# TorchIO-project/torchio

Measured on NVIDIA H100. Metric: augmented voxels/sec on 256^3 fp32 Compose pipeline, higher is better.
Workload: dtype f32

## Files before the change

### torchio_b200/csrc/fused_intensity.cu

```cuda
#include "common.cuh"
#include "tma.cuh"

namespace tio {

__device__ __forceinline__ float rician(float x, float n1, float n2) {
  float s = __fadd_rn(x, n1);
  return sqrtf(__fadd_rn(__fmul_rn(s, s), __fmul_rn(n2, n2)));
}


__device__ __forceinline__ uint4 philox4x32_10(uint4 ctr, uint2 key) {
  const uint32_t M0 = 0xD2511F53u, M1 = 0xCD9E8D57u, W0 = 0x9E3779B9u, W1 = 0xBB67AE85u;
#pragma unroll
  for (int r = 0; r < 7; ++r) {
    uint32_t hi0 = __umulhi(M0, ctr.x), lo0 = M0 * ctr.x;
    uint32_t hi1 = __umulhi(M1, ctr.z), lo1 = M1 * ctr.z;
    ctr = make_uint4(hi1 ^ ctr.y ^ key.x, lo1, hi0 ^ ctr.w ^ key.y, lo0);
    key.x += W0;
    key.y += W1;
  }
  return ctr;
}

__device__ __forceinline__ void box_muller(uint32_t a, uint32_t b, float& n0, float& n1) {
// ... 532 lines not shown
        } else {
          z1[0] = nz.z[flat];
          if (nz.rician) z2[0] = nz.z2[flat];
        }
      } else {
        const uint2 key = make_uint2((uint32_t)nz.philox_seed, (uint32_t)(nz.philox_seed >> 32));
        const uint64_t gidx = (uint64_t)(flat / V);
        uint4 rr = philox4x32_10(make_uint4((uint32_t)gidx, (uint32_t)(gidx >> 32), 0u, 0x5eedu), key);
        float nn[4];
        box_muller(rr.x, rr.y, nn[0], nn[1]);
        box_muller(rr.z, rr.w, nn[2], nn[3]);
#pragma unroll
        for (int q = 0; q < V; ++q) z1[q] = nn[q];
        if (nz.rician) {
          uint4 r2 = philox4x32_10(make_uint4((uint32_t)gidx, (uint32_t)(gidx >> 32), 1u, 0x5eedu), key);
          box_muller(r2.x, r2.y, nn[0], nn[1]);
          box_muller(r2.z, r2.w, nn[2], nn[3]);
#pragma unroll
          for (int q = 0; q < V; ++q) z2[q] = nn[q];
        }
      }
#pragma unroll
      for (int q = 0; q < V; ++q) {
        float n1 = __fadd_rn(mu, __fmul_rn(sd, z1[q]));
        if (nz.rician) v[q] = rician(v[q], n1, __fadd_rn(mu, __fmul_rn(sd, z2[q])));
        else v[q] = __fadd_rn(v[q], n1);
      }
    }
    if (gamma) {
#pragma unroll
      for (int q = 0; q < V; ++q) v[q] = signed_pow(v[q], gam);
    }
    if (V == 4) *(float4*)(y + o) = make_float4(v[0], v[1], v[2], v[3]);
    else y[o] = v[0];
  };

  if (r == 0) {
    for (int i = 0; i < I; ++i) {
      float v[V];
      load_plane(i, v);
      finish(i, v);
    }
    return;
  }

  float* mine = ring + tid * V;
  const int slot_stride = 256 * V;
  auto put = [&](int pos, const float* v) {
    int s = pos % W; if (s < 0) s += W;
    if (V == 4) *(float4*)(mine + s * slot_stride) = make_float4(v[0], v[1], v[2], v[3]);
    else mine[s * slot_stride] = v[0];
  };
  float first[V];
  load_plane(0, first);
  for (int p = -r; p <= 0; ++p) put(p, first);
  float last[V];
#pragma unroll
  for (int q = 0; q < V; ++q) last[q] = first[q];
  for (int p = 1; p < I + r; ++p) {
    if (p < I) load_plane(p, last);
    put(p, last);
    const int o = p - r;
    if (o < 0) continue;
    float acc[V];
#pragma unroll
    for (int q = 0; q < V; ++q) acc[q] = 0.0f;
    int s = (o - r) % W; if (s < 0) s += W;
    for (int t = 0; t < W; ++t) {
      const float tp = tapi[R - r + t];
      if (V == 4) {
        float4 w4 = *(const float4*)(mine + s * slot_stride);
        acc[0] = __fmaf_rn(tp, w4.x, acc[0]); acc[1] = __fmaf_rn(tp, w4.y, acc[1]);
        acc[2] = __fmaf_rn(tp, w4.z, acc[2]); acc[3] = __fmaf_rn(tp, w4.w, acc[3]);
      } else {
        acc[0] = __fmaf_rn(tp, mine[s * slot_stride], acc[0]);
      }
      if (++s == W) s = 0;
    }
    finish(o, acc);
  }
}

constexpr int M6_PF = 8;

template <bool HAS_BIAS, bool EPI>
__global__ void __launch_bounds__(256, EPI ? 1 : 2)
march6_kernel(const float* __restrict__ src, float* __restrict__ dst, int B, int C, int I, int J,
              int K, BlurArgs bl, BiasArgs bi, NoiseArgs nz, const float* __restrict__ gamma) {
  extern __shared__ __align__(16) float smem[];
  constexpr int W = 2 * F_R + 1;
  const int bc = blockIdx.z;
  const int b = bc / C;
  const int tid = threadIdx.y * blockDim.x + threadIdx.x;
  const int k = (blockIdx.x * blockDim.x + threadIdx.x) * 4;
  const int j = blockIdx.y * blockDim.y + threadIdx.y;
  const int64_t n = (int64_t)I * J * K;
  const float* x = src + (int64_t)bc * n;
  float* y = dst + (int64_t)bc * n;

  const int r = bl.taps ? bl.radius[0 * B + b] : 0;
  float* tapi = smem;
  float* g = smem + 16;
  const int ns = HAS_BIAS ? bi.si * bi.sj * bi.sk : 0;
  const bool bias_on = HAS_BIAS && !(bi.identity && bi.identity[b]);
  if (tid < W) {
    const int off = tid - F_R;
    tapi[tid] = (r > 0 && off >= -r && off <= r) ? bl.taps[((int64_t)0 * B + b) * (2 * bl.R + 1) + bl.R + off] : 0.0f;
  }
  if (bias_on) {
    const float* gs = bi.coarse + (int64_t)bc * ns;
    for (int t = tid; t < ns; t += 256) g[t] = gs[t];
  }
  __syncthreads();
  if (k >= K || j >= J) return;

  const bool noise_on = EPI && nz.mode != 0 && (!nz.keep || nz.keep[b]);
  const float mu = (EPI && nz.mode) ? nz.mean[b] : 0.0f, sd = (EPI && nz.mode) ? nz.std[b] : 0.0f;
  const float gam = (EPI && gamma) ? gamma[b] : 1.0f;
  const int gamma_mode = !(EPI && gamma) || gam == 1.0f ? 0 : (gam > 0.0f ? 1 : 2);

  LerpAxis lj, lk[4];
  int o00[4], o01[4], o10[4], o11[4];
  int cur0 = -1, cur1 = -1;
  float r_lo[4], r_hi[4];
  if (bias_on) {
    lj = lerp_axis(bi.sc_j, bi.sj, j);
#pragma unroll
    for (int v = 0; v < 4; ++v) {
      lk[v] = lerp_axis(bi.sc_k, bi.sk, k + v);
      o00[v] = lj.i0 * bi.sk + lk[v].i0; o01[v] = lj.i0 * bi.sk + lk[v].i1;
      o10[v] = lj.i1 * bi.sk + lk[v].i0; o11[v] = lj.i1 * bi.sk + lk[v].i1;
    }
  }
  const int col = j * K + k;
  const int plane = J * K;

  float4* fifo = reinterpret_cast<float4*>(g + ((ns + 3) / 4) * 4) + tid;
  auto fifo_issue = [&](int pl) {
    if (pl < I) {
      const uint32_t sa = (uint32_t)__cvta_generic_to_shared(fifo + (pl & (M6_PF - 1)) * 256);
      asm volatile("cp.async.cg.shared.global [%0], [%1], 16;" ::"r"(sa), "l"(x + (int64_t)pl * plane + col) : "memory");
    }
    asm volatile("cp.async.commit_group;" ::: "memory");
  };
#pragma unroll
  for (int pl = 0; pl < M6_PF - 1; ++pl) fifo_issue(pl);

  auto load_plane = [&](int i, float* out) {
    fifo_issue(i + M6_PF - 1);
    asm volatile("cp.async.wait_group %0;" ::"n"(M6_PF - 1) : "memory");
    const float4 t = fifo[(i & (M6_PF - 1)) * 256];
    out[0] = t.x; out[1] = t.y; out[2] = t.z; out[3] = t.w;
    if (bias_on) {
      const LerpAxis li = lerp_axis(bi.sc_i, bi.si, i);
      if (li.i0 != cur0 || li.i1 != cur1) {
        const float* p0 = g + (li.i0 * bi.sj) * bi.sk;
        const float* p1 = g + (li.i1 * bi.sj) * bi.sk;
#pragma unroll
        for (int v = 0; v < 4; ++v) {
          const float a0 = lerp2(lk[v].l0, p0[o00[v]], lk[v].l1, p0[o01[v]]);
          const float a1 = lerp2(lk[v].l0, p0[o10[v]], lk[v].l1, p0[o11[v]]);
          r_lo[v] = lerp2(lj.l0, a0, lj.l1, a1);
          const float b0 = lerp2(lk[v].l0, p1[o00[v]], lk[v].l1, p1[o01[v]]);
          const float b1 = lerp2(lk[v].l0, p1[o10[v]], lk[v].l1, p1[o11[v]]);
          r_hi[v] = lerp2(lj.l0, b0, lj.l1, b1);
        }
        cur0 = li.i0; cur1 = li.i1;
      }
#pragma unroll
      for (int v = 0; v < 4; ++v) {
        const float f = expf(lerp2(li.l0, r_lo[v], li.l1, r_hi[v]));
        out[v] = bi.divide ? __fdiv_rn(out[v], f) : __fmul_rn(out[v], f);
      }
    }
  };

  auto finish = [&](int i, float* v) {
    const int64_t o = (int64_t)i * plane + col;
    if (EPI) {
      if (noise_on) {
        const int64_t flat = (int64_t)bc * n + o;
        float z1[4], z2[4];
        if (nz.mode == 1) {
          const float4 t = __ldcs((const float4*)(nz.z + flat));
          z1[0] = t.x; z1[1] = t.y; z1[2] = t.z; z1[3] = t.w;
          if (nz.rician) {
            const float4 u = __ldcs((const float4*)(nz.z2 + flat));
            z2[0] = u.x; z2[1] = u.y; z2[2] = u.z; z2[3] = u.w;
          }
        } else {
          const uint2 key = make_uint2((uint32_t)nz.philox_seed, (uint32_t)(nz.philox_seed >> 32));
          const uint64_t gidx = (uint64_t)(flat / 4);
          uint4 rr = philox4x32_10(make_uint4((uint32_t)gidx, (uint32_t)(gidx >> 32), 0u, 0x5eedu), key);
          box_muller(rr.x, rr.y, z1[0], z1[1]);
          box_muller(rr.z, rr.w, z1[2], z1[3]);
          if (nz.rician) {
            uint4 r2 = philox4x32_10(make_uint4((uint32_t)gidx, (uint32_t)(gidx >> 32), 1u, 0x5eedu), key);
            box_muller(r2.x, r2.y, z2[0], z2[1]);
            box_muller(r2.z, r2.w, z2[2], z2[3]);
          }
        }
#pragma unroll
        for (int q = 0; q < 4; ++q) {
          const float n1 = __fadd_rn(mu, __fmul_rn(sd, z1[q]));
          if (nz.rician) v[q] = rician(v[q], n1, __fadd_rn(mu, __fmul_rn(sd, z2[q])));
          else v[q] = __fadd_rn(v[q], n1);
        }
      }
      if (gamma_mode == 1) {
#pragma unroll
        for (int q = 0; q < 4; ++q) v[q] = signed_pow_pos(v[q], gam);
      } else if (gamma_mode == 2) {
#pragma unroll
        for (int q = 0; q < 4; ++q) v[q] = signed_pow(v[q], gam);
      }
    }
    *(float4*)(y + o) = make_float4(v[0], v[1], v[2], v[3]);
  };

  if (r == 0) {
    for (int i = 0; i < I; ++i) {
      float v[4];
      load_plane(i, v);
      finish(i, v);
    }
    return;
  }

  float tp[W];
#pragma unroll
  for (int t = 0; t < W; ++t) tp[t] = tapi[t];
  float ring[W][4];
  {
    float first[4];
// ... 51 lines not shown
  const int pos = (int)((e / s) % L);
  const float* x = src + (int64_t)bc * n + (e - pos * s);
  float acc;
  if (r == 0) {
    acc = x[pos * s];
  } else {
    acc = 0.0f;
    for (int t = 0; t <= 2 * r; ++t) {
      const int q = min(max(pos - r + t, 0), L - 1);
      acc = __fmaf_rn(taps_s[t], __ldg(x + q * s), acc);
    }
  }
  const int64_t flat = (int64_t)bc * n + e;
  if (HAS_EPI) {
    if (nz.mode != 0 && (!nz.keep || nz.keep[b])) {
      const float mu = nz.mean[b], sd = nz.std[b];
      float z1, z2 = 0.0f;
      if (nz.mode == 1) {
        z1 = nz.z[flat];
        if (nz.rician) z2 = nz.z2[flat];
      } else {
        const uint2 key = make_uint2((uint32_t)nz.philox_seed, (uint32_t)(nz.philox_seed >> 32));
        float unused;
        uint4 rr = philox4x32_10(make_uint4((uint32_t)flat, (uint32_t)((uint64_t)flat >> 32), 0u, 0x77ffu), key);
        box_muller(rr.x, rr.y, z1, unused);
        if (nz.rician) box_muller(rr.z, rr.w, z2, unused);
      }
      const float n1 = __fadd_rn(mu, __fmul_rn(sd, z1));
      acc = nz.rician ? rician(acc, n1, __fadd_rn(mu, __fmul_rn(sd, z2))) : __fadd_rn(acc, n1);
    }
    if (gamma) acc = signed_pow(acc, gamma[b]);
  }
  dst[flat] = acc;
}

static inline bool aligned16f(const void* p) { return ((uintptr_t)p & 15) == 0; }

static float up_scale(int n_in, int n_out) {
  if (n_in == n_out) return 1.0f;
  return n_out > 1 ? (float)(n_in - 1) / (float)(n_out - 1) : 0.0f;
}

template <int RMAX>
static int launch_jk(const float* src, float* dst, int B, int C, int I, int J, int K,
                     const BlurArgs& bl, const NoiseArgs& nz, const float* gamma, cudaStream_t st) {
  constexpr int ROWS = A_TJ + 2 * RMAX, COLS = A_TK + 2 * RMAX, PITCH = (COLS + 3) / 4 * 4 + 4;
  const size_t smem = (size_t)(ROWS * PITCH + ROWS * A_TK + 2 * (2 * RMAX + 1)) * sizeof(float);
  const int tiles_i = (I + A_PLANES - 1) / A_PLANES;
  dim3 grid((K + A_TK - 1) / A_TK, (J + A_TJ - 1) / A_TJ, B * C * tiles_i);
  if (nz.mode != 0 || gamma) {
    if (smem > 48 * 1024)
      cudaFuncSetAttribute(jk_kernel<RMAX, true>, cudaFuncAttributeMaxDynamicSharedMemorySize, (int)smem);
    jk_kernel<RMAX, true><<<grid, 256, smem, st>>>(src, dst, B, C, I, J, K, bl, nz, gamma);
  } else {
    if (smem > 48 * 1024)
      cudaFuncSetAttribute(jk_kernel<RMAX, false>, cudaFuncAttributeMaxDynamicSharedMemorySize, (int)smem);
    jk_kernel<RMAX, false><<<grid, 256, smem, st>>>(src, dst, B, C, I, J, K, bl, nz, gamma);
  }
  return 0;
}

static int launch_march(const float* cur, float* out, int B, int C, int I, int J, int K,
                        const BiasArgs& bi, const BlurArgs& ib, const NoiseArgs& nz1,
                        const float* gamma1, cudaStream_t st, const char* who) {
  {
    const bool vec = (K % 4 == 0) && aligned16f(cur) && aligned16f(out) &&
                     (nz1.mode != 1 || (aligned16f(nz1.z) && (!nz1.z2 || aligned16f(nz1.z2))));
    const int V = vec ? 4 : 1;
    dim3 block(64, 4);
    dim3 grid((K + 64 * V - 1) / (64 * V), (J + 3) / 4, B * C);
    TIO_CHECK_ARG(grid.y <= 65535, "%s: J too large", who);
    const int R = ib.taps ? ib.R : 0;
    const int ns = bi.coarse ? bi.si * bi.sj * bi.sk : 0;
    const size_t smem = ((size_t)((2 * R + 1 + 3) / 4 * 4) + (size_t)((ns + 3) / 4 * 4) +
                         (ib.taps ? (size_t)(2 * R + 1) * 256 * V : 0)) * sizeof(float);
#define TIO_LAUNCH_MARCH(VV, BB)                                                              \
  do {                                                                                        \
    if (smem > 48 * 1024)                                                                     \
      cudaFuncSetAttribute(march_kernel<VV, BB>, cudaFuncAttributeMaxDynamicSharedMemorySize, \
                           (int)smem);                                                        \
    march_kernel<VV, BB><<<grid, block, smem, st>>>(cur, out, B, C, I, J, K, ib, bi, nz1, gamma1); \
  } while (0)
    if (vec && R <= F_R) {
      const size_t smem6 = (size_t)(16 + (ns + 3) / 4 * 4) * sizeof(float) + (size_t)M6_PF * 256 * 16;
#define TIO_LAUNCH_MARCH6(BB, EE)                                                              \
  do {                                                                                         \
    if (smem6 > 48 * 1024)                                                                     \
      cudaFuncSetAttribute(march6_kernel<BB, EE>, cudaFuncAttributeMaxDynamicSharedMemorySize, \
                           (int)smem6);                                                        \
    march6_kernel<BB, EE><<<grid, block, smem6, st>>>(cur, out, B, C, I, J, K, ib, bi, nz1, gamma1); \
  } while (0)
      const bool epi = nz1.mode != 0 || gamma1 != nullptr;
      if (bi.coarse) { if (epi) TIO_LAUNCH_MARCH6(true, true); else TIO_LAUNCH_MARCH6(true, false); }
      else { if (epi) TIO_LAUNCH_MARCH6(false, true); else TIO_LAUNCH_MARCH6(false, false); }
#undef TIO_LAUNCH_MARCH6
    } else if (vec) { if (bi.coarse) TIO_LAUNCH_MARCH(4, true); else TIO_LAUNCH_MARCH(4, false); }
    else { if (bi.coarse) TIO_LAUNCH_MARCH(1, true); else TIO_LAUNCH_MARCH(1, false); }
#undef TIO_LAUNCH_MARCH
  }
  return 0;
}

static int wide_impl(const float* src, float* dst, float* scratch, int B, int C, int I, int J,
                     int K, const BiasArgs& bi, const BlurArgs& bl, int axes_mask,
                     const NoiseArgs& nz, const float* gamma, cudaStream_t st, const char* who) {
  TIO_CHECK_ARG(bl.R <= WIDE_RMAX, "%s: blur radius R=%d > %d unsupported", who, bl.R, WIDE_RMAX);
  int axes[3], na = 0;
  for (int a : {0, 2, 1})
    if (axes_mask & (1 << a)) axes[na++] = a;
  const int steps = na + (bi.coarse ? 1 : 0);
  TIO_CHECK_ARG(src != dst && (steps < 2 || (scratch && scratch != src && scratch != dst)),
                "%s: blur radius R=%d > 16 needs src != dst and a scratch buffer", who, bl.R);
  const int64_t n = (int64_t)I * J * K;
  TIO_CHECK_ARG((n + 255) / 256 <= 0x7fffffff, "%s: volume too large", who);
  const float* cur = src;
  int left = steps;
  auto next_out = [&]() { return (--left % 2 == 0) ? dst : scratch; };
  if (bi.coarse) {
    BlurArgs none = bl;
    none.taps = nullptr;
    float* out = next_out();
    if (launch_march(cur, out, B, C, I, J, K, bi, none, NoiseArgs{}, nullptr, st, who)) return 1;
    cur = out;
  }
  const size_t smem = (size_t)(2 * bl.R + 1) * sizeof(float);
  dim3 grid((unsigned)((n + 255) / 256), B * C);
  for (int s = 0; s < na; ++s) {
    float* out = next_out();
    if (s == na - 1 && (nz.mode != 0 || gamma))
      axis_kernel<true><<<grid, 256, smem, st>>>(cur, out, B, C, I, J, K, axes[s], bl, nz, gamma);
    else
      axis_kernel<false><<<grid, 256, smem, st>>>(cur, out, B, C, I, J, K, axes[s], bl, nz, gamma);
    cur = out;
  }
  TIO_CHECK_LAUNCH();
  return 0;
}

static int fused_impl(const float* src, float* dst, float* scratch, int B, int C, int I, int J,
                      int K, BiasArgs bi, BlurArgs bl, int axes_mask, NoiseArgs nz,
                      const float* gamma, cudaStream_t st, const char* who) {
  TIO_CHECK_ARG(src && dst, "%s: null src/dst", who);
  TIO_CHECK_ARG(B > 0 && C > 0 && I > 0 && J > 0 && K > 0, "%s: bad shape", who);
  TIO_CHECK_ARG((int64_t)B * C <= 65535, "%s: B*C must be <= 65535", who);
  if (!bl.taps) axes_mask = 0;
  TIO_CHECK_ARG(!bl.taps || (bl.radius && bl.R >= 0), "%s: blur radius table missing or R=%d < 0", who, bl.R);
  if (bi.coarse) {
    bi.sc_i = up_scale(bi.si, I); bi.sc_j = up_scale(bi.sj, J); bi.sc_k = up_scale(bi.sk, K);
    TIO_CHECK_ARG((size_t)bi.si * bi.sj * bi.sk * 4 <= 64 * 1024, "%s: coarse bias grid too large", who);
  }
  if (axes_mask != 0 && bl.R > 16)
    return wide_impl(src, dst, scratch, B, C, I, J, K, bi, bl, axes_mask, nz, gamma, st, who);
  const bool need_jk = (axes_mask & 6) != 0;
  TIO_CHECK_ARG(!need_jk || (scratch && src != dst && scratch != src && scratch != dst),
                "%s: blur along J/K needs a scratch buffer and src != dst", who);
  TIO_CHECK_ARG(!((axes_mask & 1) && src == dst && !need_jk), "%s: blur along I needs src != dst", who);
  const bool need_i = (axes_mask & 1) != 0;
  const bool need_march = !need_jk || need_i || bi.coarse != nullptr;
  const float* cur = src;
  if (need_jk) {
    const int64_t tiles = (int64_t)B * C * ((I + A_PLANES - 1) / A_PLANES);
    TIO_CHECK_ARG(tiles <= 65535, "%s: batch too large for the blur grid", who);
  }
  if (need_march) {
    BlurArgs ib = bl;
    if (!need_i) ib.taps = nullptr;
    float* out = need_jk ? scratch : dst;
    if (launch_march(cur, out, B, C, I, J, K, bi, ib, need_jk ? NoiseArgs{} : nz,
                     need_jk ? nullptr : gamma, st, who))
      return 1;
    cur = out;
  }
  if (need_jk) {
    const bool tma_ok = bl.R <= F_R && (K % 4 == 0) && aligned16f(cur) && (int64_t)B * C * I < (1ll << 31);
    EncodeTiledFn encode = tma_ok ? encode_tiled_fn() : nullptr;
    CUtensorMap tm;
    bool have_map = false;
    if (encode) {
      const cuuint64_t gdim[3] = {(cuuint64_t)K, (cuuint64_t)J, (cuuint64_t)B * C * I};
      const cuuint64_t gstride[2] = {(cuuint64_t)K * 4, (cuuint64_t)J * K * 4};
      const cuuint32_t bdim[3] = {(cuuint32_t)F_COLS, (cuuint32_t)F_ROWS, 1};
      const cuuint32_t estr[3] = {1, 1, 1};
      have_map = encode(&tm, CU_TENSOR_MAP_DATA_TYPE_FLOAT32, 3, const_cast<float*>(cur), gdim, gstride,
                        bdim, estr, CU_TENSOR_MAP_INTERLEAVE_NONE, CU_TENSOR_MAP_SWIZZLE_NONE,
                        CU_TENSOR_MAP_L2_PROMOTION_L2_128B, CU_TENSOR_MAP_FLOAT_OOB_FILL_NONE) == CUDA_SUCCESS;
    }
    if (have_map) {
      const int tiles_i = (I + A_PLANES - 1) / A_PLANES;
      dim3 grid((K + A_TK - 1) / A_TK, (J + A_TJ - 1) / A_TJ, B * C * tiles_i);
      if (nz.mode != 0 || gamma) {
        cudaFuncSetAttribute(jk6_kernel<true>, cudaFuncAttributeMaxDynamicSharedMemorySize, (int)F_SMEM);
        jk6_kernel<true><<<grid, 256, F_SMEM, st>>>(tm, dst, B, C, I, J, K, bl, nz, gamma);
      } else {
        cudaFuncSetAttribute(jk6_kernel<false>, cudaFuncAttributeMaxDynamicSharedMemorySize, (int)F_SMEM);
        jk6_kernel<false><<<grid, 256, F_SMEM, st>>>(tm, dst, B, C, I, J, K, bl, nz, gamma);
      }
    } else if (bl.R <= F_R) {
      launch_jk<6>(cur, dst, B, C, I, J, K, bl, nz, gamma, st);
    } else {
      launch_jk<16>(cur, dst, B, C, I, J, K, bl, nz, gamma, st);
    }
  }
  TIO_CHECK_LAUNCH();
  return 0;
}

}

using namespace tio;

extern "C" int tio_blur(const float* src, float* dst, float* scratch, int B, int C, int I, int J,
                        int K, const float* taps, const int32_t* radius, int R, int axes_mask,
                        const uint8_t* identity, void* stream) {
  (void)identity;
  TIO_CHECK_ARG(taps && radius, "tio_blur: null taps/radius");
  TIO_CHECK_ARG(src != dst, "tio_blur: src and dst must not alias");
  BiasArgs bi{};
  BlurArgs bl{taps, radius, R};
  NoiseArgs nz{};
  return fused_impl(src, dst, scratch, B, C, I, J, K, bi, bl, axes_mask & 7, nz, nullptr,
                    (cudaStream_t)stream, "tio_blur");
}

extern "C" int tio_intensity_fused(const float* src, float* dst, float* scratch, int B, int C,
                                   int I, int J, int K, const float* coarse, int si, int sj,
                                   int sk, const uint8_t* bias_identity, int bias_divide,
                                   const float* taps, const int32_t* radius, int R,
                                   int axes_mask, const float* mean, const float* std,
                                   const uint8_t* keep, const float* z, const float* z2,
                                   uint64_t philox_seed, int noise_mode, int rician_flag,
                                   const float* gamma, void* stream) {
  BiasArgs bi{};
  bi.coarse = coarse; bi.identity = bias_identity; bi.si = si; bi.sj = sj; bi.sk = sk;
  bi.divide = bias_divide;
  BlurArgs bl{taps, radius, R};
  NoiseArgs nz{};
  nz.mode = noise_mode;
  TIO_CHECK_ARG(noise_mode >= 0 && noise_mode <= 2, "tio_intensity_fused: bad noise_mode");
  if (noise_mode) {
    TIO_CHECK_ARG(mean && std, "tio_intensity_fused: noise needs mean/std");
    TIO_CHECK_ARG(noise_mode != 1 || (z && (!rician_flag || z2)), "tio_intensity_fused: normals missing");
// ... 7 lines not shown
```

### torchio_b200/ops.py

```python

from __future__ import annotations

import os
import threading

import numpy as np
import torch
from torch import Tensor

from . import _native, tables

DTYPE_CODES = {
    torch.float32: 0, torch.uint8: 1, torch.int8: 2,
    torch.int16: 3, torch.int32: 4, torch.int64: 5,
}
NEAREST, LINEAR, LABEL_PV = 0, 1, 2
FLAG_PASSTHROUGH, FLAG_ELASTIC = 1, 2

_counter = threading.local()


def launches() -> int:
    return getattr(_counter, "n", 0)

# ... 195 lines not shown
    fill = torch.empty(c, dtype=torch.float32, device=src.device)
    with torch.cuda.device(src.device):
        _native.call("tio_min_sample0", _ptr(src), c, n, _ptr(fill), _stream(src))
    _count(2)
    return fill


def crop_patches(volume: Tensor, corners, size, out: Tensor | None = None) -> Tensor:
    _require_cuda(volume, "crop_patches")
    if volume.ndim != 4:
        raise ValueError(f"crop_patches expects a (C, I, J, K) volume, got {tuple(volume.shape)}")
    volume = volume.contiguous()
    corners = np.ascontiguousarray(np.asarray(corners, dtype=np.int32).reshape(-1, 3))
    n = corners.shape[0]
    c, i, j, k = (int(v) for v in volume.shape)
    pi, pj, pk = (int(v) for v in size)
    if n == 0:
        return volume.new_empty((0, c, pi, pj, pk))
    if corners.min() < 0 or np.any(corners + np.asarray([pi, pj, pk]) > np.asarray([i, j, k])):
        raise ValueError("crop_patches: a patch extends beyond the volume")
    (corners_d,) = upload(volume.device, corners)
    if out is None:
        dst = torch.empty((n, c, pi, pj, pk), dtype=volume.dtype, device=volume.device)
    else:
        dst = out
        if (tuple(dst.shape) != (n, c, pi, pj, pk) or dst.dtype != volume.dtype or dst.device != volume.device
                or not dst.is_contiguous()):
            raise ValueError("crop_patches: `out` must be a contiguous (n, C, *size) block of the volume's dtype/device")
    with torch.cuda.device(volume.device):
        _native.call(
            "tio_crop_patches", _ptr(volume), _ptr(dst), volume.element_size(), c, i, j, k, n,
            _ptr(corners_d), pi, pj, pk, _stream(volume),
        )
    _count(1)
    return dst


PAD_MODES = {"constant": 0, "replicate": 1, "reflect": 2, "circular": 3}


def remap(src: Tensor, out_shape, offsets, *, mode: str = "constant", fill=0, flip: Tensor | None = None,
          out: Tensor | None = None) -> Tensor:
    _require_cuda(src, "remap")
    if src.ndim != 5:
        raise ValueError(f"remap expects (B, C, I, J, K), got {tuple(src.shape)}")
    src = src.contiguous()
    b, c, i, j, k = (int(v) for v in src.shape)
    oi, oj, ok = (int(v) for v in out_shape)
    if out is None:
        dst = torch.empty((b, c, oi, oj, ok), dtype=src.dtype, device=src.device)
    else:
        dst = out
        if (tuple(dst.shape) != (b, c, oi, oj, ok) or dst.dtype != src.dtype or dst.device != src.device
                or not dst.is_contiguous()):
            raise ValueError("remap: `out` must be a contiguous (B, C, *out_shape) block of the source's dtype/device")
    fill_host = torch.tensor([fill]).to(src.dtype)
    with torch.cuda.device(src.device):
        _native.call(
            "tio_remap", _ptr(src), _ptr(dst), src.element_size(), b, c, i, j, k, oi, oj, ok,
            int(offsets[0]), int(offsets[1]), int(offsets[2]), PAD_MODES[mode],
            fill_host.data_ptr(), _ptr(flip), _stream(src),
        )
    _count(1)
    return dst


def blur(src: Tensor, taps: Tensor, radius: Tensor, big_r: int, axes_mask: int,
         identity: Tensor | None) -> Tensor:
    _require_cuda(src, "blur")
    src = src.contiguous()
    b, c, i, j, k = src.shape
    dst = torch.empty_like(src)
    scratch = torch.empty_like(src) if (axes_mask & 6) or big_r > WIDE_R else None
    with torch.cuda.device(src.device):
        _native.call(
            "tio_blur", _ptr(src), _ptr(dst), _ptr(scratch), b, c, i, j, k, _ptr(taps),
            _ptr(radius), int(big_r), int(axes_mask), _ptr(identity), _stream(src),
        )
    _count(_fused_launches(axes_mask, False, big_r))
    return dst


WIDE_R = 16


def _fused_launches(axes_mask: int, has_bias: bool, big_r: int = 0) -> int:
    if axes_mask & 7 and big_r > WIDE_R:
        return bin(axes_mask & 7).count("1") + int(has_bias)
    jk = bool(axes_mask & 6)
    march = (not jk) or bool(axes_mask & 1) or has_bias
    return int(jk) + int(march)


def moments(values: Tensor, mask: Tensor | None = None) -> tuple[float, float, float]:
    _require_cuda(values, "moments")
    values = values.contiguous()
    m8 = None if mask is None else mask.expand_as(values).contiguous().to(torch.uint8)
    out = torch.empty(3, dtype=torch.float64, device=values.device)
    with torch.cuda.device(values.device):
        _native.call("tio_moments", _ptr(values), _ptr(m8), values.numel(), _ptr(out), _stream(values))
    _count(1)
    s, ss, n = out.tolist()
    return s, ss, n


def quantile_neighbours(values: Tensor, qs, mask: Tensor | None = None):
    _require_cuda(values, "quantile_neighbours")
    values = values.contiguous()
    m8 = None if mask is None else mask.expand_as(values).contiguous().to(torch.uint8)
    qs = np.ascontiguousarray(np.asarray(qs, dtype=np.float64).reshape(-1))
    m = int(qs.shape[0])
    dev = values.device
    vals = torch.empty(2 * m, dtype=torch.float32, device=dev)
    out = torch.empty(m + 1, dtype=torch.float64, device=dev)
    ws_bytes = _native.lib().tio_quantiles_workspace_bytes()
    ws = torch.empty(ws_bytes, dtype=torch.uint8, device=dev)
    with torch.cuda.device(dev):
        _native.call("tio_quantiles", _ptr(values), _ptr(m8), values.numel(), qs.ctypes.data, m, _ptr(vals),
                     _ptr(out), out[m:].data_ptr(), _ptr(ws), ws_bytes, _stream(values))
    _count(7)
    host = out.tolist()
    return vals.tolist(), host[:m], int(host[m])


def quantiles_batched(values: Tensor, qs, mask: Tensor | None = None):
    _require_cuda(values, "quantiles_batched")
    if values.dtype not in RESOLUTION_DTYPE_CODES:
        raise TypeError(f"quantiles_batched: unsupported dtype {values.dtype}")
    values = values.contiguous()
    b = values.shape[0]
    per_elem = values[0].numel()
    m8 = None if mask is None else mask.expand_as(values).contiguous().to(torch.uint8)
    qs = np.ascontiguousarray(np.asarray(qs, dtype=np.float64).reshape(-1))
    m = int(qs.shape[0])
    dev = values.device
    vals = torch.empty((b, 2 * m), dtype=torch.float32, device=dev)
    weights = torch.empty((b, m), dtype=torch.float64, device=dev)
    count = torch.empty(b, dtype=torch.float64, device=dev)
    has_nan = torch.empty(b, dtype=torch.uint8, device=dev)
    ws_bytes = _native.lib().tio_quantiles_batched_workspace_bytes(b, m)
    ws = torch.empty(ws_bytes, dtype=torch.uint8, device=dev)
    with torch.cuda.device(dev):
        _native.call("tio_quantiles_batched", _ptr(values), RESOLUTION_DTYPE_CODES[values.dtype], _ptr(m8), b,
                     per_elem, qs.ctypes.data, m, _ptr(vals), _ptr(weights), _ptr(count), _ptr(has_nan), _ptr(ws),
                     ws_bytes, _stream(values))
    _count(2 + 5 * ((m + 12) // 13))
    return vals, weights, count, has_nan


def histogram_tables(values: Tensor, weights: Tensor, has_nan: Tensor, landmarks: Tensor) -> Tensor:
    b, m = weights.shape
    landmarks = landmarks.to(device=values.device, dtype=torch.float32).contiguous()
    tables = torch.empty((b, 3 * (m - 1)), dtype=torch.float32, device=values.device)
    with torch.cuda.device(values.device):
        _native.call("tio_histogram_tables", _ptr(values), _ptr(weights), _ptr(has_nan), _ptr(landmarks), b, m,
                     _ptr(tables), _stream(values))
    _count(1)
    return tables


def histogram_map(data: Tensor, tables: Tensor, m: int) -> None:
    _require_cuda(data, "histogram_map")
    if data.dtype not in RESOLUTION_DTYPE_CODES:
        raise TypeError(f"histogram_map: unsupported dtype {data.dtype}")
    if not data.is_contiguous():
        raise ValueError("histogram_map: data must be contiguous")
    if data.numel() == 0:
        return
    with torch.cuda.device(data.device):
        _native.call("tio_histogram_map", _ptr(data), _ptr(data), RESOLUTION_DTYPE_CODES[data.dtype], data.shape[0],
                     data[0].numel(), _ptr(tables), int(m), _stream(data))
    _count(1)


def rescale(src: Tensor, *, lo: float | None = None, hi: float | None = None, sub=None, div=None, mul=None,
            add=None, keep=None) -> Tensor:
    _require_cuda(src, "rescale")
    src = src.contiguous()
    b = src.shape[0]
    flags = (1 if lo is not None else 0)
    tabs = []
    for bit, table in ((2, sub), (4, div), (8, mul), (16, add)):
        if table is None:
            tabs.append(None)
            continue
        flags |= bit
        arr = np.asarray(table, dtype=np.float32).reshape(-1)
        tabs.append(np.ascontiguousarray(np.broadcast_to(arr, (b,)) if arr.size == 1 else arr))
    keep_np = None if keep is None else np.ascontiguousarray(np.asarray(keep, dtype=np.uint8))
    sub_d, div_d, mul_d, add_d, keep_d = upload(src.device, *tabs, keep_np)
    dst = torch.empty_like(src)
    with torch.cuda.device(src.device):
        _native.call("tio_rescale", _ptr(src), _ptr(dst), b, src[0].numel(),
                     float(lo if lo is not None else 0.0), float(hi if hi is not None else 0.0),
                     _ptr(sub_d), _ptr(div_d), _ptr(mul_d), _ptr(add_d), _ptr(keep_d), flags, _stream(src))
    _count(2)
    return dst


def intensity_fused(
    src: Tensor, *, coarse: Tensor | None = None, bias_identity: Tensor | None = None,
    bias_divide: bool = False, taps: Tensor | None = None, radius: Tensor | None = None,
    big_r: int = 0, axes_mask: int = 0, mean: Tensor | None = None, std: Tensor | None = None,
    keep: Tensor | None = None, z: Tensor | None = None, z2: Tensor | None = None,
    philox_seed: int = 0, noise_mode: int = 0, rician: bool = False,
    gamma: Tensor | None = None,
) -> Tensor:
    _require_cuda(src, "intensity_fused")
    src = src.contiguous()
    b, c, i, j, k = src.shape
    dst = torch.empty_like(src)
    jk = taps is not None and ((axes_mask & 6) or (axes_mask & 7 and big_r > WIDE_R))
    scratch = torch.empty_like(src) if jk else None
    si = sj = sk = 0
    if coarse is not None:
        si, sj, sk = coarse.shape[2:]
    with torch.cuda.device(src.device):
        _native.call(
            "tio_intensity_fused", _ptr(src), _ptr(dst), _ptr(scratch), b, c, i, j, k,
            _ptr(coarse), si, sj, sk, _ptr(bias_identity), int(bool(bias_divide)),
            _ptr(taps), _ptr(radius), int(big_r), int(axes_mask),
            _ptr(mean), _ptr(std), _ptr(keep), _ptr(z), _ptr(z2),
            int(philox_seed) & (2**64 - 1), int(noise_mode), int(bool(rician)),
            _ptr(gamma), _stream(src),
        )
    _count(_fused_launches(axes_mask if taps is not None else 0, coarse is not None, big_r))
    return dst



_MT_TABLE_FILE = _native.LIB_PATH.parent / "mt19937_jump.bin"
_mt_host_table: Tensor | None = None
_mt_device_tables: dict = {}
_mt_lock = threading.Lock()
MT_MAX_WORDS = 1 << 31
MT_TABLE_HEADER = (0x4D544A31, 21, 16, 64, 78, 10496)


def mt19937_host_table() -> Tensor:
    global _mt_host_table
    with _mt_lock:
        if _mt_host_table is None:
            lib = _native.lib()
            nbytes = lib.tio_mt19937_table_bytes()
            blob = None
            if _MT_TABLE_FILE.exists() and _MT_TABLE_FILE.stat().st_size == nbytes:
                cached = np.fromfile(_MT_TABLE_FILE, dtype=np.uint8)
                if tuple(int(v) for v in cached[:24].view(np.uint32)) == MT_TABLE_HEADER:
                    blob = torch.from_numpy(cached)
            if blob is None:
                blob = torch.zeros(nbytes, dtype=torch.uint8)
                _native.call("tio_mt19937_build_table", blob.data_ptr(), nbytes)
                try:
                    blob.numpy().tofile(_MT_TABLE_FILE)
                except OSError:
                    pass
            _mt_host_table = blob
        return _mt_host_table


def _mt_table(device: torch.device) -> Tensor:
    key = (device.type, device.index)
    table = _mt_device_tables.get(key)
    if table is None:
        with _init_lock:
            table = _mt_device_tables.get(key)
            if table is None:
                table = mt19937_host_table().to(device)
                torch.cuda.synchronize(device)
                _mt_device_tables[key] = table
    return table


def randn_mt19937(seed: int, offset: int, n: int, device, out: Tensor | None = None) -> Tensor:
    device = torch.device(device)
    if n < 16 or n % 16 or offset % 16 or offset + n > MT_MAX_WORDS:
        raise ValueError("randn_mt19937: offset and n must be multiples of 16, n >= 16,"
                         " offset + n <= 2**31")
    z = torch.empty(n, dtype=torch.float32, device=device) if out is None else out
    lib = _native.lib()
    ws_bytes = lib.tio_randn_mt19937_workspace_bytes(offset, n)
    workspace = torch.empty(ws_bytes, dtype=torch.uint8, device=device)
    table = _mt_table(device)
    with torch.cuda.device(device):
        _native.call("tio_randn_mt19937", int(seed) & 0xFFFFFFFF, offset, n, _ptr(z), _ptr(table),
                     _ptr(workspace), ws_bytes, torch.cuda.current_stream(device).cuda_stream)
    _count(4)
    return z



_cuda_rng_lock = threading.Lock()


def labels_to_image(labels: Tensor, label_values, means, stds, draw=None) -> Tensor:
    if labels.dtype not in DTYPE_CODES:
# ... 239 lines not shown
```

### torchio_b200/transforms/intensity.py

```python

from __future__ import annotations

import os
import warnings
from typing import Any

import numpy as np
import torch
from torch import Tensor

from .. import ops, tables
from ..data import ImagesBatch, LabelMap, ScalarImage, SubjectsBatch
from ..params import to_nonneg_range, to_range
from .base import IntensityTransform, Transform, chunk_info, staged_derived


def _as_f32(data: Tensor) -> Tensor:
    return data if data.dtype == torch.float32 else data.float()




class BiasField(IntensityTransform):
    def __init__(self, *, std=0.5, scale: float = 0.025, **kwargs: Any) -> None:
        super().__init__(**kwargs)
        self.std = to_nonneg_range(std)
        if scale <= 0 or scale > 1:
            raise ValueError(f"scale must be in (0, 1], got {scale}")
        self.scale = scale

    @property
    def supports_per_instance_params(self) -> bool:
        return True

    @property
    def supports_per_instance_p(self) -> bool:
        return True

    def supports_chunks(self, batch: SubjectsBatch) -> bool:
        return True

    def make_params(self, batch: SubjectsBatch) -> dict[str, Any]:
        n = self._resolve_n(batch)
        if n is None:
            std = self.std.sample_1d()
            seed = int(torch.randint(0, 2**31, (1,)).item())
            return {"std": std, "seed": seed, "scale": self.scale}
        keep = self._keep_mask(batch, n)
        std = self._mask_identity(self.std.sample_1d(n), keep, identity=0.0)
        seeds = [int(torch.randint(0, 2**31, (1,)).item()) for _ in range(n)]
        params = {"std": self._serialize_param(std), "seed": seeds, "scale": self.scale}
        self._tag_batched(params, batch, n, keep, ["std", "seed"])
        return params

    def apply_transform(self, batch: SubjectsBatch, params: dict[str, Any]) -> SubjectsBatch:
        _apply_bias(self, batch, params["std"], params["seed"], params["scale"], divide=False)
        return batch

    @property
    def invertible(self) -> bool:
        return True

    def inverse(self, params: dict[str, Any]) -> _BiasFieldInverse:
        return _BiasFieldInverse(std=params["std"], seed=params["seed"], scale=params["scale"],
                                 copy=False)


def _bias_stage(data_shape, affines, std, seed, scale, *, divide: bool):
    per_element = isinstance(std, list)
    if (not per_element and std == 0) or (per_element and all(s == 0 for s in std)):
        return None
    b = data_shape[0]
    if per_element and len(std) != b:
        raise RuntimeError(
            f"Per-instance parameters were recorded for {len(std)} elements"
            f" but the batch has {b}"
        )
    info = chunk_info()
    if info is not None and not per_element:
        full = tables.coarse_bias_fields((info.total, *data_shape[1:]), std, seed, scale)
        coarse = full[info.b0:info.b1].contiguous()
    else:
        coarse = tables.coarse_bias_fields(data_shape, std, seed, scale)
    return {
        "coarse": coarse,
        "bias_identity": np.asarray([s == 0 for s in std], dtype=np.uint8) if per_element else None,
# ... 78 lines not shown
    t = tables.blur_tables(vox, ib.data.shape[0])
    if t is None:
        return None
    return {"taps": t.taps, "radius": t.radius, "big_r": t.big_r, "axes_mask": t.axes_mask}




def _noise_mode() -> str:
    mode = os.environ.get("TIO_B200_NOISE", "exact").lower()
    if mode not in ("exact", "philox"):
        raise ValueError(f"TIO_B200_NOISE must be 'exact' or 'philox', got {mode!r}")
    return mode


class Noise(IntensityTransform):
    def __init__(self, *, mean=0.0, std=0.25, rician: bool = False, **kwargs: Any) -> None:
        super().__init__(**kwargs)
        self.mean = to_range(mean)
        self.std = to_nonneg_range(std)
        self.rician = rician

    @property
    def supports_per_instance_params(self) -> bool:
        return True

    @property
    def supports_per_instance_p(self) -> bool:
        return True

    def supports_chunks(self, batch: SubjectsBatch) -> bool:
        if _noise_mode() != "exact":
            return False
        images = self._get_images(batch).values()
        words = sum(int(np.prod(ib.data.shape)) for ib in images) * (2 if self.rician else 1)
        if words > ops.MT_MAX_WORDS:
            return False
        return all(int(np.prod(ib.data.shape[1:])) % 16 == 0 for ib in images)

    def make_params(self, batch: SubjectsBatch) -> dict[str, Any]:
        seed = int(torch.randint(0, 2**31, (1,)).item())
        n = self._resolve_n(batch)
        keep = self._keep_mask(batch, n)
        mean = self._mask_identity(self.mean.sample_1d(n), keep, identity=0.0)
        std = self._mask_identity(self.std.sample_1d(n), keep, identity=0.0)
        params = {
            "mean": self._serialize_param(mean), "std": self._serialize_param(std),
            "seed": seed, "rician": self.rician,
        }
        self._tag_batched(params, batch, n, keep, ["mean", "std"])
        return params

    def apply_transform(self, batch: SubjectsBatch, params: dict[str, Any]) -> SubjectsBatch:
        run_stages(self._get_images(batch), [_noise_stage_factory(params)])
        return batch


def _noise_stage_factory(params):
    mode = _noise_mode()
    generator = torch.Generator(device="cpu")
    generator.manual_seed(params["seed"])
    rician = bool(params.get("rician", False))
    keep = params.get("_keep")

    consumed = [0]

    def draw(shape, device):
        n = int(np.prod(shape))
        info = chunk_info()
        if info is None:
            start, n_full = consumed[0], n
        else:
            per = n // shape[0]
            start, n_full = consumed[0] + per * info.b0, per * info.total
        on_device = (not ragged[0] and n >= 16 and n % 16 == 0 and start % 16 == 0
                     and n_full % 16 == 0 and start + n <= ops.MT_MAX_WORDS
                     and device.type == "cuda")
        if info is not None and not on_device:
            raise RuntimeError("Noise: this batch cannot be streamed in slices (ragged normal stream)")
        if n_full < 16 or n_full % 16:
            ragged[0] = True
        consumed[0] += n_full + (16 if (n_full >= 16 and n_full % 16) else 0)
        if on_device:
            return ops.randn_mt19937(params["seed"], start, n, device).view(shape), None
        if host_state[0] != start:
            skip = start - host_state[0]
            if skip % 16 == 0 and skip >= 16:
                torch.randn(skip, generator=generator)
            else:
                raise RuntimeError("Noise: cannot realign the host generator (ragged stream)")
        pin = torch.cuda.is_available()
        z = torch.empty(shape, dtype=torch.float32, pin_memory=pin)
        torch.randn(shape, generator=generator, out=z)
        host_state[0] = consumed[0]
        return None, z

    host_state = [0]
    ragged = [False]

    def stage(ib, index):
        shape = ib.data.shape
        b = shape[0]
        out = {
            "mean": tables.per_element_vector(params["mean"], b),
            "std": tables.per_element_vector(params["std"], b),
            "keep": None if keep is None else np.asarray(keep, dtype=np.uint8),
            "rician": rician,
        }
        if mode == "philox":
            out["noise_mode"] = 2
            out["philox_seed"] = (int(params["seed"]) << 8) | (index & 0xFF)
            return out
        out["noise_mode"] = 1
        z_dev, z_host = draw(shape, ib.data.device)
        out["z" if z_dev is not None else "z_host"] = z_dev if z_dev is not None else z_host
        if rician:
            z_dev, z_host = draw(shape, ib.data.device)
            out["z2" if z_dev is not None else "z2_host"] = z_dev if z_dev is not None else z_host
        return out

    return stage




class Gamma(IntensityTransform):
    def __init__(self, *, log_gamma=0.0, **kwargs: Any) -> None:
        super().__init__(**kwargs)
        self.log_gamma = to_range(log_gamma)
        self._warn_if_noop(is_noop=self.log_gamma.is_constant(0.0), hint="log_gamma=(-0.3, 0.3)")

    @property
    def supports_per_instance_params(self) -> bool:
        return True

    @property
    def supports_per_instance_p(self) -> bool:
        return True

    def supports_chunks(self, batch: SubjectsBatch) -> bool:
        return True

    def make_params(self, batch: SubjectsBatch) -> dict[str, Any]:
        n = self._resolve_n(batch)
        keep = self._keep_mask(batch, n)
        log_gamma = self._mask_identity(self.log_gamma.sample_1d(n), keep, identity=0.0)
        params = {"log_gamma": self._serialize_param(log_gamma)}
        self._tag_batched(params, batch, n, keep, ["log_gamma"])
        return params

    def apply_transform(self, batch: SubjectsBatch, params: dict[str, Any]) -> SubjectsBatch:
        _apply_gamma(self, batch, params["log_gamma"])
        return batch

    @property
    def invertible(self) -> bool:
        return True

    def inverse(self, params: dict[str, Any]) -> _GammaInverse:
        return _GammaInverse(log_gamma=params["log_gamma"], copy=False)


def _apply_gamma(transform, batch, log_gamma) -> None:
    run_stages(transform._get_images(batch),
               [lambda ib, index: {"gamma": tables.gamma_values(log_gamma, ib.data.shape[0])}])


class _GammaInverse(IntensityTransform):
    def __init__(self, *, log_gamma, **kwargs: Any) -> None:
        super().__init__(**kwargs)
        self._log_gamma = log_gamma

    def apply_transform(self, batch: SubjectsBatch, params: dict[str, Any]) -> SubjectsBatch:
        lg = self._log_gamma
        _apply_gamma(self, batch, [-v for v in lg] if isinstance(lg, list) else -lg)
        return batch




class LabelsToImage(Transform):

    def __init__(self, label_key: str | None = None, *, image_key: str = "image_from_labels", mean=None,
                 std=None, default_mean=(0.1, 0.9), default_std=(0.01, 0.1), ignore_background: bool = False,
                 **kwargs: Any) -> None:
        super().__init__(**kwargs)
        self.label_key = label_key
        self.image_key = image_key
        self.mean_ranges = [to_range(m) for m in mean] if mean is not None else None
        self.std_ranges = [to_range(s) for s in std] if std is not None else None
        self.default_mean = to_range(default_mean)
        self.default_std = to_range(default_std)
        self.ignore_background = ignore_background

    @property
    def supports_per_instance_params(self) -> bool:
        return True

    def make_params(self, batch: SubjectsBatch) -> dict[str, Any]:
        _, label_batch = self._find_label_batch(batch)
        unique = sorted(int(v) for v in label_batch.data[0].unique().tolist())
# ... 218 lines not shown
        return True

    def inverse(self, params: dict[str, Any]) -> _RescaleInverse:
        return _RescaleInverse(out_min=params["out_min"], out_max=params["out_max"], in_min=params.get("in_min"),
                               in_max=params.get("in_max"), in_ranges=params.get("in_ranges"), copy=False)


RescaleIntensity = Normalize
ZNormalization = Standardize


def _value_range(value):
    if isinstance(value, (int, float)):
        return to_range(float(value))
    if isinstance(value, (tuple, list)):
        return to_range(tuple(float(v) for v in value))
    return to_range(value)


def _out_min_and_range(out_min, out_max):
    if isinstance(out_min, list):
        lo = np.asarray(out_min, dtype=np.float32)
        return lo, (np.asarray(out_max, dtype=np.float32) - lo).astype(np.float32)
    return out_min, out_max - out_min


class _RescaleInverse(IntensityTransform):
    def __init__(self, *, out_min, out_max, in_min, in_max, in_ranges, **kwargs: Any) -> None:
        super().__init__(**kwargs)
        self._out_min, self._out_max = out_min, out_max
        self._in_min, self._in_max, self._in_ranges = in_min, in_max, in_ranges

    def make_params(self, batch: SubjectsBatch) -> dict[str, Any]:
        return {}

    def apply_transform(self, batch: SubjectsBatch, params: dict[str, Any]) -> SubjectsBatch:
        for name, img_batch in self._get_images(batch).items():
            if self._in_min is not None and self._in_max is not None:
                in_min, in_max = self._in_min, self._in_max
            elif self._in_ranges is not None and name in self._in_ranges:
                in_min, in_max = self._in_ranges[name]
            else:
                continue
            in_range = in_max - in_min
            if in_range == 0:
                continue
            out_min, out_range = _out_min_and_range(self._out_min, self._out_max)
            keep = None
            if isinstance(out_range, float):
                if out_range == 0:
                    continue
            else:
                keep = (out_range != 0).astype(np.uint8)
                out_range = np.where(out_range == 0, np.float32(1.0), out_range)
            data = _as_f32(img_batch.data)
            img_batch.data = ops.rescale(data, sub=out_min, div=out_range, mul=in_range, add=in_min, keep=keep)
        return batch


class _Staged:

    def __init__(self, img_batch) -> None:
        self.img_batch = img_batch

    def __enter__(self):
        data = self.img_batch.data
        if data.is_cuda:
            return self.img_batch
        from .base import execution_device

        class _View:
            pass

        view = _View()
        view.data = data[:1].to(execution_device(), non_blocking=True)
        return view

    def __exit__(self, *exc) -> None:
        return None



_TABLE_KEYS = ("coarse", "bias_identity", "taps", "radius", "mean", "std", "keep", "gamma")


def run_stages(images, stage_builders) -> None:
    for index, ib in enumerate(images.values()):
        kwargs: dict[str, Any] = {}
        for build in stage_builders:
            stage = build(ib, index)
            if stage:
                kwargs.update(stage)
        if not kwargs:
            continue
        data = ib.data
        device = data.device
        uploaded = ops.upload(device, *[kwargs.get(k) for k in _TABLE_KEYS])
        for key, value in zip(_TABLE_KEYS, uploaded, strict=True):
            if key in kwargs:
                kwargs[key] = value
        z_host, z2_host = kwargs.pop("z_host", None), kwargs.pop("z2_host", None)
        if z_host is not None:
            kwargs["z"] = z_host.to(device, non_blocking=True)
        if z2_host is not None:
            kwargs["z2"] = z2_host.to(device, non_blocking=True)
        out = ops.intensity_fused(_as_f32(data), **kwargs)
        promotes = ("gamma" in kwargs or "mean" in kwargs) and data.dtype != torch.float64
        ib.data = out if promotes or out.dtype == data.dtype else out.to(data.dtype)
```

Measured before the change: 50.54 billion.

## Overlap device normal generation with first fused pass on side stream; shrink march6 blocks

```diff
diff --git a/torchio_b200/csrc/fused_intensity.cu b/torchio_b200/csrc/fused_intensity.cu
--- a/torchio_b200/csrc/fused_intensity.cu
+++ b/torchio_b200/csrc/fused_intensity.cu
@@ -638,9 +638,10 @@
 }
 
 constexpr int M6_PF = 8;
+constexpr int M6_THREADS = 128;
 
 template <bool HAS_BIAS, bool EPI>
-__global__ void __launch_bounds__(256, EPI ? 1 : 2)
+__global__ void __launch_bounds__(M6_THREADS, EPI ? 2 : 4)
 march6_kernel(const float* __restrict__ src, float* __restrict__ dst, int B, int C, int I, int J,
               int K, BlurArgs bl, BiasArgs bi, NoiseArgs nz, const float* __restrict__ gamma) {
   extern __shared__ __align__(16) float smem[];
@@ -665,7 +666,7 @@
   }
   if (bias_on) {
     const float* gs = bi.coarse + (int64_t)bc * ns;
-    for (int t = tid; t < ns; t += 256) g[t] = gs[t];
+    for (int t = tid; t < ns; t += M6_THREADS) g[t] = gs[t];
   }
   __syncthreads();
   if (k >= K || j >= J) return;
@@ -694,7 +695,7 @@
   float4* fifo = reinterpret_cast<float4*>(g + ((ns + 3) / 4) * 4) + tid;
   auto fifo_issue = [&](int pl) {
     if (pl < I) {
-      const uint32_t sa = (uint32_t)__cvta_generic_to_shared(fifo + (pl & (M6_PF - 1)) * 256);
+      const uint32_t sa = (uint32_t)__cvta_generic_to_shared(fifo + (pl & (M6_PF - 1)) * M6_THREADS);
       asm volatile("cp.async.cg.shared.global [%0], [%1], 16;" ::"r"(sa), "l"(x + (int64_t)pl * plane + col) : "memory");
     }
     asm volatile("cp.async.commit_group;" ::: "memory");
@@ -705,7 +706,7 @@
   auto load_plane = [&](int i, float* out) {
     fifo_issue(i + M6_PF - 1);
     asm volatile("cp.async.wait_group %0;" ::"n"(M6_PF - 1) : "memory");
-    const float4 t = fifo[(i & (M6_PF - 1)) * 256];
+    const float4 t = fifo[(i & (M6_PF - 1)) * M6_THREADS];
     out[0] = t.x; out[1] = t.y; out[2] = t.z; out[3] = t.w;
     if (bias_on) {
       const LerpAxis li = lerp_axis(bi.sc_i, bi.si, i);
@@ -923,13 +924,16 @@
     march_kernel<VV, BB><<<grid, block, smem, st>>>(cur, out, B, C, I, J, K, ib, bi, nz1, gamma1); \
   } while (0)
     if (vec && R <= F_R) {
-      const size_t smem6 = (size_t)(16 + (ns + 3) / 4 * 4) * sizeof(float) + (size_t)M6_PF * 256 * 16;
+      const size_t smem6 = (size_t)(16 + (ns + 3) / 4 * 4) * sizeof(float) + (size_t)M6_PF * M6_THREADS * 16;
+      const dim3 block6(64, M6_THREADS / 64);
+      const dim3 grid6(grid.x, (J + block6.y - 1) / block6.y, grid.z);
+      TIO_CHECK_ARG(grid6.y <= 65535, "%s: J too large", who);
 #define TIO_LAUNCH_MARCH6(BB, EE)                                                              \
   do {                                                                                         \
     if (smem6 > 48 * 1024)                                                                     \
       cudaFuncSetAttribute(march6_kernel<BB, EE>, cudaFuncAttributeMaxDynamicSharedMemorySize, \
                            (int)smem6);                                                        \
-    march6_kernel<BB, EE><<<grid, block, smem6, st>>>(cur, out, B, C, I, J, K, ib, bi, nz1, gamma1); \
+    march6_kernel<BB, EE><<<grid6, block6, smem6, st>>>(cur, out, B, C, I, J, K, ib, bi, nz1, gamma1); \
   } while (0)
       const bool epi = nz1.mode != 0 || gamma1 != nullptr;
       if (bi.coarse) { if (epi) TIO_LAUNCH_MARCH6(true, true); else TIO_LAUNCH_MARCH6(true, false); }
@@ -993,11 +997,12 @@
   if (axes_mask != 0 && bl.R > 16)
     return wide_impl(src, dst, scratch, B, C, I, J, K, bi, bl, axes_mask, nz, gamma, st, who);
   const bool need_jk = (axes_mask & 6) != 0;
-  TIO_CHECK_ARG(!need_jk || (scratch && src != dst && scratch != src && scratch != dst),
-                "%s: blur along J/K needs a scratch buffer and src != dst", who);
-  TIO_CHECK_ARG(!((axes_mask & 1) && src == dst && !need_jk), "%s: blur along I needs src != dst", who);
   const bool need_i = (axes_mask & 1) != 0;
   const bool need_march = !need_jk || need_i || bi.coarse != nullptr;
+  TIO_CHECK_ARG(!need_jk || src != dst, "%s: blur along J/K needs src != dst", who);
+  TIO_CHECK_ARG(!(need_jk && need_march) || (scratch && scratch != src && scratch != dst),
+                "%s: bias or blur along I followed by blur along J/K needs a scratch buffer", who);
+  TIO_CHECK_ARG(!((axes_mask & 1) && src == dst && !need_jk), "%s: blur along I needs src != dst", who);
   const float* cur = src;
   if (need_jk) {
     const int64_t tiles = (int64_t)B * C * ((I + A_PLANES - 1) / A_PLANES);
diff --git a/torchio_b200/ops.py b/torchio_b200/ops.py
--- a/torchio_b200/ops.py
+++ b/torchio_b200/ops.py
@@ -301,6 +301,7 @@
 
 
 WIDE_R = 16
+MARCH6_R = 6
 
 
 def _fused_launches(axes_mask: int, has_bias: bool, big_r: int = 0) -> int:
@@ -429,8 +430,10 @@
     src = src.contiguous()
     b, c, i, j, k = src.shape
     dst = torch.empty_like(src)
-    jk = taps is not None and ((axes_mask & 6) or (axes_mask & 7 and big_r > WIDE_R))
-    scratch = torch.empty_like(src) if jk else None
+    wide = taps is not None and bool(axes_mask & 7) and big_r > WIDE_R
+    jk = taps is not None and bool(axes_mask & 6)
+    first = coarse is not None or (taps is not None and bool(axes_mask & 1))
+    scratch = torch.empty_like(src) if wide or (jk and first) else None
     si = sj = sk = 0
     if coarse is not None:
         si, sj, sk = coarse.shape[2:]
diff --git a/torchio_b200/transforms/intensity.py b/torchio_b200/transforms/intensity.py
--- a/torchio_b200/transforms/intensity.py
+++ b/torchio_b200/transforms/intensity.py
@@ -2,6 +2,7 @@
 from __future__ import annotations
 
 import os
+import threading
 import warnings
 from typing import Any
 
@@ -246,7 +247,7 @@
             ragged[0] = True
         consumed[0] += n_full + (16 if (n_full >= 16 and n_full % 16) else 0)
         if on_device:
-            return ops.randn_mt19937(params["seed"], start, n, device).view(shape), None
+            return (lambda: ops.randn_mt19937(params["seed"], start, n, device).view(shape)), None
         if host_state[0] != start:
             skip = start - host_state[0]
             if skip % 16 == 0 and skip >= 16:
@@ -276,11 +277,15 @@
             out["philox_seed"] = (int(params["seed"]) << 8) | (index & 0xFF)
             return out
         out["noise_mode"] = 1
-        z_dev, z_host = draw(shape, ib.data.device)
-        out["z" if z_dev is not None else "z_host"] = z_dev if z_dev is not None else z_host
-        if rician:
-            z_dev, z_host = draw(shape, ib.data.device)
-            out["z2" if z_dev is not None else "z2_host"] = z_dev if z_dev is not None else z_host
+        replays = []
+        for key in ("z", "z2") if rician else ("z",):
+            replay, z_host = draw(shape, ib.data.device)
+            if replay is not None:
+                replays.append((key, replay))
+            else:
+                out[key + "_host"] = z_host
+        if replays:
+            out["z_replay"] = replays
         return out
 
     return stage
@@ -665,6 +670,29 @@
 
 
 _TABLE_KEYS = ("coarse", "bias_identity", "taps", "radius", "mean", "std", "keep", "gamma")
+_BIAS_KEYS = ("coarse", "bias_identity", "bias_divide")
+_replay_local = threading.local()
+
+
+def _replay_stream(device) -> torch.cuda.Stream:
+    cache = getattr(_replay_local, "streams", None)
+    if cache is None:
+        cache = _replay_local.streams = {}
+    key = (device.type, device.index)
+    stream = cache.get(key)
+    if stream is None:
+        stream = cache[key] = torch.cuda.Stream(device=device,
+                                                priority=torch.cuda.Stream.priority_range()[1])
+    return stream
+
+
+def _overlaps_pass1(kwargs, src: Tensor) -> bool:
+    if kwargs.get("taps") is None or not kwargs.get("axes_mask", 0) & 6:
+        return False
+    if kwargs.get("coarse") is None and not kwargs["axes_mask"] & 1:
+        return False
+    return (kwargs["big_r"] <= ops.MARCH6_R and src.shape[-1] % 4 == 0
+            and src.data_ptr() % 16 == 0)
 
 
 def run_stages(images, stage_builders) -> None:
@@ -678,6 +706,20 @@
             continue
         data = ib.data
         device = data.device
+        src = _as_f32(data)
+        replays = kwargs.pop("z_replay", [])
+        forked = bool(replays) and _overlaps_pass1(kwargs, src)
+        if forked:
+            current = torch.cuda.current_stream(device)
+            side = _replay_stream(device)
+            side.wait_stream(current)
+            with torch.cuda.stream(side):
+                for key, replay in replays:
+                    kwargs[key] = replay()
+                normals_ready = side.record_event()
+        else:
+            for key, replay in replays:
+                kwargs[key] = replay()
         uploaded = ops.upload(device, *[kwargs.get(k) for k in _TABLE_KEYS])
         for key, value in zip(_TABLE_KEYS, uploaded, strict=True):
             if key in kwargs:
@@ -687,6 +729,17 @@
             kwargs["z"] = z_host.to(device, non_blocking=True)
         if z2_host is not None:
             kwargs["z2"] = z2_host.to(device, non_blocking=True)
-        out = ops.intensity_fused(_as_f32(data), **kwargs)
+        if forked:
+            blur = {k: kwargs[k] for k in ("taps", "radius", "big_r")}
+            bias = {k: kwargs[k] for k in _BIAS_KEYS if k in kwargs}
+            rest = {k: v for k, v in kwargs.items() if k not in _BIAS_KEYS and k not in blur}
+            first = ops.intensity_fused(src, **bias, **blur, axes_mask=kwargs["axes_mask"] & 1)
+            current.wait_event(normals_ready)
+            for key, _ in replays:
+                kwargs[key].record_stream(current)
+            rest["axes_mask"] = kwargs["axes_mask"] & 6
+            out = ops.intensity_fused(first, **blur, **rest)
+        else:
+            out = ops.intensity_fused(src, **kwargs)
         promotes = ("gamma" in kwargs or "mean" in kwargs) and data.dtype != torch.float64
         ib.data = out if promotes or out.dtype == data.dtype else out.to(data.dtype)
```

New measurement: 52.96 billion (median of 6 runs). 4.8% higher.
